# DavidRother/cooking_zoo

Measured on AMD Instinct MI355X. Metric: env-steps/sec at N parallel envs (1/2/4/8 GPU) + achieved HBM GB/s, higher is better.
Workload: dtype u8/u32 state, f64 obs+reward

## Files before the change

### cooking_zoo_amd/_native.py

```python
from __future__ import annotations

import ctypes as C
import os
import sys

_HERE = os.path.dirname(os.path.abspath(__file__))
LIB_PATH = os.environ.get("CZ_LIB", os.path.join(_HERE, "csrc", "libcookingzoo_hip.so"))
HEADER_PATH = os.path.join(os.path.dirname(_HERE), "include", "cookingzoo.h")


def header_abi_version() -> int:
    import re
    if os.path.exists(HEADER_PATH):
        m = re.search(r"^#define\s+CZ_ABI_VERSION\s+(\d+)", open(HEADER_PATH).read(), flags=re.M)
        if not m:
            raise NativeError(f"no CZ_ABI_VERSION in {HEADER_PATH}")
        return int(m.group(1))
    try:
        from cooking_zoo_amd._abi import CZ_ABI_VERSION
    except ImportError as exc:
        raise NativeError(f"neither {HEADER_PATH} nor cooking_zoo_amd/_abi.py (generated by `make -C cooking_zoo_amd/csrc`) is "
                          f"there: the expected ABI number of libcookingzoo_hip.so is unknown") from exc
    return int(CZ_ABI_VERSION)

# ... 82 lines not shown
    ("cz_load_partner_table", C.c_int, [_VP, _VP, _I32]),
    ("cz_load_layout_ranks", C.c_int, [_VP, _I32, _I32, _VP]),
    ("cz_load_goal_table", C.c_int, [_VP, _VP, _I32, _I32]),
    ("cz_num_goals", _I32, [_VP]),
    ("cz_set_tasks_device", C.c_int, [_VP, _VP, _VP, _VP, _I32, _U64]),
    ("cz_set_tasks_refused", _I64, [_VP]),
    ("cz_infos_device", C.c_int, [_VP, _I64, _I64, _VP, _VP, _VP, _VP, _VP]),
    ("cz_num_actions", _I32, [_VP]),
    ("cz_action_effects_device", C.c_int, [_VP, _I64, _I64, _U32, _U32, _VP, _VP]),
    ("cz_render_sprites", _I32, []),
    ("cz_load_sprites", C.c_int, [_VP, _VP, _I32, _I32]),
    ("cz_render_device", C.c_int, [_VP, _I64, _I64, _I32, _U32, _VP, _VP]),
    ("cz_obs_table_f32", C.c_int, [_VP, _VP]),
    ("cz_codes_pitch", _I32, [_VP]),
    ("cz_obs_table", C.c_int, [_VP, _VP]),
    ("cz_obs_table_device", _VP, [_VP]),
    ("cz_probe_closed_loop_compact", C.c_int, [_VP, _I32, _I32, _VP, _VP, _VP, _VP, _VP, C.POINTER(C.c_float)]),
    ("cz_step_device_many", C.c_int, [_VP, _I32, _VP, _I64, _I32, _VP, _VP, _VP, _VP]),
    ("cz_step_device_ring", C.c_int, [_VP, _I32, _VP, _I64, _I32, _I32, _VP, _VP, _VP, _VP]),
    ("cz_ring_prepare", C.c_int, [_VP, _I32, _VP, _I64, _I32, _I32, _VP, _VP, _VP, _VP]),
    ("cz_launch_counts", C.c_int, [_VP, C.POINTER(_I64), C.POINTER(_I64), _I32]),
    ("cz_set_ring_fused", C.c_int, [_VP, _I32]),
    ("cz_ring_fused_steps", C.c_int64, [_VP, _I32]),
    ("cz_last_marks", C.c_int, [_VP, _VP]),
    ("cz_set_stream", C.c_int, [_VP, _VP]),
    ("cz_probe_output_only", C.c_int, [_VP, _VP, C.c_size_t, _I32, _VP]),
    ("cz_probe_policy", C.c_int, [_VP, _VP, _VP, _VP]),
    ("cz_probe_closed_loop", C.c_int, [_VP, _I32, _I32, _VP, _VP, _VP, _VP, _VP, C.POINTER(C.c_float)]),
    ("cz_rollout", C.c_int, [_VP, _I32, _U64, _U32, _VP, _VP, _VP, _VP]),
    ("cz_rollout_compact", C.c_int, [_VP, _I32, _U64, _U32, _VP, _VP, _VP, _VP, _VP]),
    ("cz_rollout_actions", C.c_int, [_VP, _I32, _VP, _VP, _VP, _VP, _VP]),
    ("cz_rollout_f32", C.c_int, [_VP, _I32, _U64, _U32, _VP, _VP, _VP, _VP]),
    ("cz_rollout_actions_f32", C.c_int, [_VP, _I32, _VP, _VP, _VP, _VP, _VP]),
    ("cz_action", _U32, [_U64, _I64, _I32, _U32, _U32]),
    ("cz_next_layout", _U32, [_I64, _U32, _U32, _U32]),
    ("cz_next_layout_group", _U32, [_I64, _U32, _U32, _U32, _U32, _U32]),
    ("cz_dev_alloc", _VP, [_VP, C.c_size_t]),
    ("cz_dev_free", C.c_int, [_VP, _VP]),
    ("cz_host_alloc", _VP, [_VP, C.c_size_t]),
    ("cz_host_free", C.c_int, [_VP, _VP]),
    ("cz_memcpy_h2d", C.c_int, [_VP, _VP, _VP, C.c_size_t]),
    ("cz_memcpy_d2h", C.c_int, [_VP, _VP, _VP, C.c_size_t]),
    ("cz_timer_start", C.c_int, [_VP]),
    ("cz_timer_stop", C.c_int, [_VP, C.POINTER(C.c_float)]),
    ("cz_kernel_time_reset", C.c_int, [_VP, _I32]),
    ("cz_kernel_time_read", C.c_int, [_VP, C.POINTER(C.c_double), C.POINTER(_I64)]),
    ("cz_get_stats", C.c_int, [_VP, C.POINTER(CzStats)]),
    ("cz_reset_stats", C.c_int, [_VP]),
    ("cz_episodes_collect", C.c_int, [_VP, _VP, _VP, _VP, _VP, _VP, _I32, _VP]),
    ("cz_comm_unique_id", C.c_int, [_VP]),
    ("cz_comm_init", C.c_int, [_VP, _I32, _I32, _VP]),
    ("cz_stats_allgather", C.c_int, [_VP, _VP]),
    ("cz_comm_barrier", C.c_int, [_VP]),
    ("cz_runtime_paths", C.c_int, [C.c_char_p, C.c_char_p, C.c_size_t]),
]

ADDED_SYMBOLS = frozenset(["cz_rollout_f32", "cz_rollout_actions_f32", "cz_reset_device", "cz_reset_device_refused",
                           "cz_episodes_collect", "cz_sizeof_episode", "cz_save_device", "cz_restore_device", "cz_restore_device_refused",
                           "cz_observe_grid_device", "cz_grid_channels", "cz_navigate_device", "cz_nav_max_targets", "cz_partner_device",
                           "cz_partner_bad_recipes", "cz_partner_row_words", "cz_load_partner_table", "cz_load_layout_ranks", "cz_num_actions",
                           "cz_action_effects_device", "cz_render_sprites", "cz_load_sprites", "cz_render_device", "cz_load_goal_table", "cz_num_goals",
                           "cz_set_tasks_device", "cz_set_tasks_refused", "cz_infos_device"])

_lib = None
_absent = frozenset()


def _missing(name):
    def call(*args):
        raise NativeError(f"{LIB_PATH} does not export {name}: it was built before that entry point was added - rebuild it "
                          f"(make -C cooking_zoo_amd/csrc)")
    return call


class NativeError(RuntimeError):
    pass


class _LateTorchGuard:

    MESSAGE = ("`import torch` after cooking_zoo_amd has loaded libcookingzoo_hip.so: torch's bundled ROCm runtime would be loaded next "
               "to the system one already in use and the process would abort at exit. Import torch BEFORE creating the first "
               "cooking_zoo_amd environment (see INTEGRATION.md), or set CZ_ALLOW_LATE_TORCH=1 to take the risk.")

    class _Refuse:
# ... 65 lines not shown
```

### cooking_zoo_amd/csrc/cz_api.hip

```cpp
#include <hip/hip_runtime.h>
#include <dlfcn.h>
#include <stdarg.h>
#include <stdio.h>
#include <stdlib.h>
#include <string.h>

#include <atomic>
#include <string>
#include <vector>

#include "../../include/cookingzoo.h"
#include "cz_launch.h"
#include "cz_generate.h"

using namespace cz;

constexpr int STAT_CHAINS = 256, STAT_COLS = 13;
__global__ __launch_bounds__(64) void k_stats_chains(const uint32_t *__restrict__ su, const double *__restrict__ sf,
                                                     const uint32_t *__restrict__ state, int RW, int N,
                                                     unsigned long long *__restrict__ part ) {
    const int chain = (int)blockIdx.x * 4 + ((int)threadIdx.x >> 4), col = (int)threadIdx.x & 15;
    const int widx = col == 0 ? (int)SU_STEPS : col == 1 ? (int)SU_EPISODES : col == 2 ? (int)SU_LENSUM : col == 3 ? (int)SU_TRUNC
                   : col == 4 ? (int)SU_TERM : col < 9 ? (int)SU_COMPLETED0 + col - 5 : 0;
    const int fidx = (col >= 9 && col < STAT_COLS) ? (int)SF_SUM0 + col - 9 : (int)SF_SUM0;
// ... 242 lines not shown
    void *d_sprites = nullptr;
    int32_t sprites_M = 0;
    double obs_table[LUT_SIZE];
    int32_t *d_reset_words = nullptr;
    unsigned long long *d_reset_refused = nullptr;
    unsigned long long *d_restore_refused = nullptr;
    unsigned long long *d_tasks_refused = nullptr;
    uint8_t *d_goal = nullptr;
    int n_goal_rows = 0;
    int num_goals = 0;
    uint8_t *codes = nullptr;
    float *obs32 = nullptr;
    void *d_codes_stage = nullptr;
    void *d_dump = nullptr;
    int32_t *d_actions = nullptr;
    double *d_obs = nullptr;
    char *d_small = nullptr, *h_small = nullptr;
    uint32_t *h_marks = nullptr, *d_marks_mapped = nullptr;
    std::vector<uint32_t> last_marks;
    char *h_stage = nullptr, *d_stage = nullptr;
    struct RingKey {
        const int32_t *ring = nullptr; int64_t stride = 0; int32_t period = 0;
        double *obs = nullptr, *rew = nullptr; uint8_t *term = nullptr, *trunc = nullptr; hipStream_t stream = nullptr; uint64_t version = 0;
        bool operator==(const RingKey &o) const {
            return ring == o.ring && stride == o.stride && period == o.period && obs == o.obs && rew == o.rew && term == o.term &&
                   trunc == o.trunc && stream == o.stream && version == o.version;
        }
    } ring_key;
    struct RunGraph { int32_t slot, len; hipGraphExec_t ge; uint64_t used; };
    std::vector<RunGraph> ring_graphs;
    uint64_t ring_clock = 0;
    int64_t n_graph_kernels = 0, n_direct_kernels = 0;
    uint64_t tables_version = 0;
    hipEvent_t ev0 = nullptr, ev1 = nullptr;
    bool ktime = false;
    std::vector<hipEvent_t> kev;
    size_t kev_used = 0;
    double ktime_ms = 0.0;
    int64_t klaunches = 0;
    void *rccl = nullptr;
    void *comm = nullptr;
    int n_ranks = 1, rank = 0;
    int wt_override = -1;
    bool lean_enabled = true;
    bool lean_cfg_enabled = true;
    int last_step_variant = -1;
    int last_step_lean = -1;
    int last_step_mode = -1;
    bool huge = false;
    int instance = 0;
    unsigned long long *tl_base = nullptr;
    int32_t tl_cap = 0;
    int64_t tl_count = 0;
    bool graphs_enabled = true;
    bool ring_fused = false;
    int64_t n_ring_fused_steps = 0;
    int32_t graph_min_run = 48;
    int32_t ring_prefix = 0;
    size_t zero_copy_bytes = (size_t)256 << 10;
    cz_stats *d_gather = nullptr;
    std::string err;
};

static thread_local std::string g_err;
static int ready(cz_handle h);
static int set_device(cz_handle h);
static int begin_ranged_call(cz_handle h, int64_t b, int64_t c);
static void mark_ranks(cz_handle h, int32_t first, int32_t count, int ok);
static int flush_updates(cz_handle h, bool force);

static int fail(cz_handle h, const char *fmt, ...) {
    char buf[512];
    va_list ap;
    va_start(ap, fmt);
    vsnprintf(buf, sizeof buf, fmt, ap);
    va_end(ap);
    if (h) h->err = buf; else g_err = buf;
    return 1;
}

#define HIPCHK(h, call)                                                                      \
// ... 105 lines not shown
    CREATE_CHK(hipStreamCreateWithFlags(&h->own_stream, hipStreamNonBlocking));
    h->stream = h->own_stream;
    CREATE_CHK(hipEventCreate(&h->ev0));
    CREATE_CHK(hipEventCreate(&h->ev1));
    Params &P = h->P;
    memset(&P, 0, sizeof P);
    P.N = cfg->num_envs; P.A = cfg->num_agents; P.W = cfg->width; P.H = cfg->height; P.D = cfg->max_dyn; P.F = cfg->feat_len;
    const int CW = (C + 3) / 4;
    P.dyn0_off = CELL_WORD0 + CW;
    P.dyn1_off = P.dyn0_off + P.D;
    P.RW = (P.dyn1_off + P.D + 15) / 16 * 16;
    P.scheme = cfg->action_scheme; P.max_steps = cfg->max_steps; P.end_all = cfg->end_condition_all ? 1 : 0;
    P.R = cfg->num_recipes; P.auto_reset = cfg->auto_reset ? 1 : 0; P.env_id_base = cfg->env_id_base;
    P.recipe_reward = cfg->recipe_reward; P.recipe_penalty = cfg->recipe_penalty; P.node_reward = cfg->recipe_node_reward;
    P.time_penalty_step = cfg->max_time_penalty / (double)cfg->max_steps;
    P.T = 1;
    if (const char *s = getenv("CZ_WT")) h->wt_override = atoi(s);
    if (const char *s = getenv("CZ_LEAN")) h->lean_enabled = atoi(s) != 0;
    if (const char *s = getenv("CZ_LEAN_CFG")) h->lean_cfg_enabled = atoi(s) != 0;
    if (const char *s = getenv("CZ_GRAPHS")) h->graphs_enabled = atoi(s) != 0;
    if (const char *s = getenv("CZ_GRAPH_MIN_RUN")) h->graph_min_run = atoi(s) < 4 ? 4 : (atoi(s) > 256 ? 256 : atoi(s));
    if (const char *s = getenv("CZ_RING_PREFIX")) h->ring_prefix = atoi(s) < 0 ? 0 : (atoi(s) > 16 ? 16 : atoi(s));
    if (const char *s = getenv("CZ_ZERO_COPY_BYTES")) h->zero_copy_bytes = (size_t)atoll(s);
#ifdef CZ_SMALL_ONLY
    if (!(P.D <= 64 && C <= 64)) { fail(nullptr, "cz_create: this diagnostic library holds the small kernel instance only"); cz_destroy(h); return 1; }
    h->kl = launchers_small();
#else
    h->instance = (P.D <= 64 && C <= 64) ? 0 : (P.D <= 128 && C <= 256) ? 1 : 2;
    h->kl = h->instance == 0 ? launchers_small() : h->instance == 1 ? launchers_large() : launchers_huge();
#endif
    h->huge = P.D > 128 || C > 256;
    {
        double x = 0.0;
        x += (double)0 * P.node_reward;
        x += 0.0 * P.recipe_reward;
        x += 0.0 * P.recipe_penalty;
        x += P.time_penalty_step;
        P.reward_idle = x;
    }
    const size_t N = (size_t)P.N;
    const size_t state_bytes = N * P.RW * 4;
    CREATE_CHK(hipMalloc(&h->d_state, state_bytes));
    CREATE_CHK(hipMemsetAsync(h->d_state, 0, state_bytes, h->stream));
    CREATE_CHK(hipMalloc(&h->d_stat_u, N * SU_WORDS * 4));
    CREATE_CHK(hipMalloc(&h->d_stat_f, N * SF_WORDS * 8));
    CREATE_CHK(hipMemsetAsync(h->d_stat_u, 0, N * SU_WORDS * 4, h->stream));
// ... 52 lines not shown
        CREATE_CHK(hipMemcpy(h->d_lut, lut, sizeof lut, hipMemcpyHostToDevice));
        CREATE_CHK(hipMemcpy((char *)h->d_lut + sizeof lut, submask, sizeof submask, hipMemcpyHostToDevice));
        P.lut = h->d_lut;
        memcpy(h->obs_table, lut, sizeof lut);
    }
#undef CREATE_CHK
    *out = h;
    return 0;
}

extern "C" int cz_destroy(cz_handle h) {
    if (!h) return 0;
    (void)hipSetDevice(h->cfg.device_id);
    (void)hipStreamSynchronize(h->stream);
    if (h->comm && h->rccl) {
        typedef int (*destroy_t)(void *);
        destroy_t f = (destroy_t)dlsym(h->rccl, "ncclCommDestroy");
        if (f) f(h->comm);
    }
    void *ptrs[] = {h->d_codes_stage, h->d_spawn_tables, h->d_gen_tables, h->d_reset_words, h->d_reset_refused, h->d_restore_refused, h->d_tasks_refused, h->d_goal, h->d_dump, h->d_lut, h->d_sprites, h->d_state, h->d_lay_block, h->d_lay_desc, h->d_lay_rank, h->d_partner, h->d_recipes, h->d_stat_u, h->d_stat_f, h->d_ep_seen, h->d_ep_blocks, h->d_stats_out, h->d_stats_part,
                    h->d_actions, h->d_obs, h->d_small, h->d_gather};
    for (void *p : ptrs)
        if (p) (void)hipFree(p);
    for (auto &r : h->ring_graphs)
        if (r.ge) (void)hipGraphExecDestroy(r.ge);
    if (h->copy_stream) { (void)hipStreamSynchronize(h->copy_stream); (void)hipStreamDestroy(h->copy_stream); }
    if (h->ev_copy_done) (void)hipEventDestroy(h->ev_copy_done);
    if (h->ev_steps_issued) (void)hipEventDestroy(h->ev_steps_issued);
    if (h->ev_main_copy_done) (void)hipEventDestroy(h->ev_main_copy_done);
    if (h->h_lay_stage) (void)hipHostFree(h->h_lay_stage);
    if (h->rank_stream) { (void)hipStreamSynchronize(h->rank_stream); (void)hipStreamDestroy(h->rank_stream); }
    if (h->ev_rank_done) (void)hipEventDestroy(h->ev_rank_done);
    if (h->h_rank_stage) (void)hipHostFree(h->h_rank_stage);
    if (h->h_stage) (void)hipHostFree(h->h_stage);
    if (h->h_small) (void)hipHostFree(h->h_small);
    if (h->h_marks) (void)hipHostFree(h->h_marks);
    for (hipEvent_t e : h->kev) (void)hipEventDestroy(e);
    if (h->ev0) (void)hipEventDestroy(h->ev0);
    if (h->ev1) (void)hipEventDestroy(h->ev1);
    if (h->own_stream) (void)hipStreamDestroy(h->own_stream);
    delete h;
    return 0;
}

extern "C" int cz_set_stream(cz_handle h, void *hip_stream) {
    if (!h) return fail(nullptr, "null handle");
    HIPCHK(h, hipSetDevice(h->cfg.device_id));
    HIPCHK(h, hipStreamSynchronize(h->stream));
    h->stream = hip_stream ? (hipStream_t)hip_stream : h->own_stream;
    h->tables_version++;
    return 0;
}
extern "C" int cz_set_spawn(cz_handle h, double despawn_rate, double respawn_rate, int32_t grace_period, uint64_t seed,
                            int32_t n_levels, const uint8_t *level_of_layout, int32_t stride, const uint8_t *spawn_x, const int32_t *n_x,
                            const uint8_t *spawn_y, const int32_t *n_y) {
// ... 505 lines not shown
        if (c.obs) return "float32 observation rows are switched on (cz_set_f32_output): pass d_obs = NULL, or switch them off "
                          "with cz_set_f32_output(h, NULL) to get float64 rows";
    }
    form = obs32 ? OBS_F32 : codes ? OBS_CODES : OBS_F64;
    P = h->P;
    P.actions = c.actions; P.obs = c.obs; P.rewards = c.rewards; P.term = c.term; P.trunc = c.trunc; P.marks_out = c.marks;
    P.T = c.T; P.seed = c.seed; P.step0 = c.step0;
    if (obs32) P.obs32 = obs32; else P.codes = codes;
    return nullptr;
}

static hipError_t choose_step(cz_handle h, const Params &P, bool fused, ObsForm form, StepChoice &c) {
    c.lean = false;
    c.cfg = -1;
    if (fused && form == OBS_F32) c.mode = P.actions ? ROLLOUT_ACTIONS_F32 : ROLLOUT_F32;
    else if (fused) c.mode = P.actions ? ROLLOUT_ACTIONS : form != OBS_CODES ? ROLLOUT : P.obs ? ROLLOUT_CODES : ROLLOUT_CODES_ONLY;
    else c.mode = form == OBS_F32 ? STEP_F32 : form == OBS_CODES ? STEP_CODES : STEP;
    if (c.mode == STEP)
        c.lean = h->lean_enabled && h->kl.has_lean && P.obs && !P.marks_out && !P.wide && !(P.auto_reset & 2) && P.F <= 128 * OBS_PAIRS && P.wt == 1;
    if (c.lean && h->lean_cfg_enabled) c.cfg = lean_cfg_of(P);
    return !fused && !P.actions ? hipErrorInvalidValue : hipSuccess;
}

static int launch_step(cz_handle h, const StepCall &call) {
    if ((h->P.auto_reset & 2) && h->spawn_layouts != h->n_layouts)
        return fail(h, "despawn / respawn is on, but the layout pool was reloaded since cz_set_spawn (now %d layouts): call cz_set_spawn "
                       "again (it maps every layout to the level whose spawn areas it uses)", h->n_layouts);
    const hipStream_t stream = h->stream;
    const bool fused = call.fused;
    Params P;
    ObsForm form;
    if (const char *refused = resolve_step(h, call, P, form)) return fail(h, "%s", refused);
    const bool f32 = form == OBS_F32;
    const size_t obs_bytes = (size_t)P.N * P.A * P.F * (f32 ? 4 : 8);
    if (!fused) P.wt = obs_bytes > ((size_t)224 << 20) ? 2 : P.N <= 10240 ? 1 : 0;
    else P.wt = (obs_bytes > ((size_t)224 << 20) && (size_t)P.F * (f32 ? 4 : 8) >= 4096) ? 2 : 0;
    if (h->wt_override >= 0) P.wt = h->wt_override;
    if (!fused) {
        if (!P.rewards) P.rewards = (double *)h->d_dump;
        if (!P.term) P.term = (uint8_t *)h->d_dump;
        if (!P.trunc) P.trunc = (uint8_t *)h->d_dump;
    }
#ifdef CZ_TIMELINE
    P.timeline = (h->tl_base && h->tl_cap > 0) ? h->tl_base + (size_t)(h->tl_count++ % h->tl_cap) * (size_t)P.N * 2 : nullptr;
#endif
    hipEvent_t e0 = nullptr, e1 = nullptr;
    if (h->ktime && caller_capturing(h)) return fail(h, "kernel timing (cz_kernel_time_reset) cannot run inside a stream capture of the caller");
    if (h->ktime) {
        while (h->kev.size() < h->kev_used + 2) {
            hipEvent_t e;
            HIPCHK(h, hipEventCreate(&e));
            h->kev.push_back(e);
        }
        e0 = h->kev[h->kev_used]; e1 = h->kev[h->kev_used + 1];
        h->kev_used += 2;
        HIPCHK(h, hipEventRecord(e0, stream));
    }
    StepChoice choice;
    const hipError_t chosen = choose_step(h, P, fused, form, choice);
    h->last_step_lean = choice.lean ? 1 : 0;
    h->last_step_mode = choice.mode;
    h->last_step_variant = !choice.lean ? -1 : choice.cfg < 0 ? 0 : (0x100 | P.R | (P.end_all << 4) | (P.walk_touches << 5));
    HIPCHK(h, chosen);
    HIPCHK(h, h->kl.step(P, stream, choice));
    if (h->ktime) HIPCHK(h, hipEventRecord(e1, stream));
    return 0;
}
extern "C" int cz_reset(cz_handle h, int64_t b, int64_t c, const int32_t *layout_ids, const uint8_t *recipe_ids,
                        const uint32_t *pool_words, double *obs) {
    if (ready(h) || check_range(h, b, c)) return 1;
    if (c == 0) return 0;
    if (!layout_ids || !recipe_ids) return fail(h, "cz_reset: null argument");
    HIPCHK(h, hipSetDevice(h->cfg.device_id));
    std::vector<uint32_t> pools((size_t)c, 0u);
    for (int64_t i = 0; i < c; ++i) {
        if (layout_ids[i] < 0 || layout_ids[i] >= h->n_layouts) return fail(h, "cz_reset: layout id %d out of range", layout_ids[i]);
        for (int r = 0; r < h->P.R; ++r)
            if (recipe_ids[i * 4 + r] >= h->n_recipes) return fail(h, "cz_reset: recipe id %d out of range", recipe_ids[i * 4 + r]);
        if (pool_words) {
            uint32_t base = pool_words[i] & 0xFFFFu, count = pool_words[i] >> 16;
            if (count && (int)(base + count) > h->n_layouts) return fail(h, "cz_reset: layout pool slice [%u,%u) out of range", base, base + count);
            pools[(size_t)i] = pool_words[i];
        }
    }
    int32_t *const d_lay = h->d_reset_words;
    uint32_t *const d_rec = (uint32_t *)h->d_reset_words + h->P.N, *const d_pool = (uint32_t *)h->d_reset_words + 2 * (size_t)h->P.N;
    HIPCHK(h, hipMemcpyAsync(d_lay, layout_ids, (size_t)c * 4, hipMemcpyHostToDevice, h->stream));
// ... 378 lines not shown
extern "C" int cz_diag_read_layout_pool(cz_handle h, int32_t first, int32_t count, uint32_t *records, uint32_t *desc) {
    if (ready(h)) return 1;
    if (!h->d_lay_init || !h->d_lay_desc) return fail(h, "cz_diag_read_layout_pool: no layout pool loaded");
    if (first < 0 || count < 0 || (int64_t)first + count > h->n_layouts)
        return fail(h, "cz_diag_read_layout_pool: slots [%d, %d) outside the resident pool of %d layouts", first, first + count, h->n_layouts);
    if (count == 0) return 0;
    if (set_device(h)) return 1;
    HIPCHK(h, hipStreamSynchronize(h->stream));
    if (records)
        HIPCHK(h, hipMemcpy(records, h->d_lay_init + (size_t)first * h->P.RW, (size_t)count * h->P.RW * 4, hipMemcpyDeviceToHost));
    if (desc)
        HIPCHK(h, hipMemcpy(desc, h->d_lay_desc + (size_t)first * h->P.F, (size_t)count * h->P.F * 4, hipMemcpyDeviceToHost));
    return 0;
}
extern "C" int cz_obs_table(cz_handle h, double *table) {
    if (!h || !table) return fail(h, "cz_obs_table: null argument");
    memcpy(table, h->obs_table, sizeof h->obs_table);
    return 0;
}
extern "C" const void *cz_obs_table_device(cz_handle h) { return h ? (const void *)h->d_lut : nullptr; }

static bool ring_fusable(cz_handle h, const StepCall &c, int32_t K, int64_t stride);
static int launch_ring_fused(cz_handle h, const StepCall &c, int32_t K, const int32_t *d_ring, int64_t stride, int32_t period, int32_t first_slot);
extern "C" int cz_step_device_many(cz_handle h, int32_t K, const int32_t *d_actions, int64_t action_stride, int32_t action_period,
                                   double *d_obs, double *d_rewards, uint8_t *d_term, uint8_t *d_trunc) {
    if (begin_device_call(h, d_actions && K >= 1 && action_period >= 1, "cz_step_device_many: bad arguments")) return 1;
    StepCall c{d_actions, d_obs, d_rewards, d_term, d_trunc};
    if (ring_fusable(h, c, K, action_stride)) return launch_ring_fused(h, c, K, d_actions, action_stride, action_period, 0);
    for (int32_t k = 0; k < K; ++k) {
        c.actions = d_actions + (int64_t)(k % action_period) * action_stride;
        if (launch_step(h, c)) return 1;
    }
    return 0;
}

constexpr int RING_MAX_GRAPH = 256, RING_CACHE = 64;
static int ring_capture(cz_handle h, StepCall &c, const int32_t *d_ring, int64_t stride, int32_t slot, int32_t len, hipGraphExec_t &ge) {
    hipGraph_t g = nullptr;
    HIPCHK(h, hipStreamBeginCapture(h->stream, hipStreamCaptureModeThreadLocal));
    int bad = 0;
    for (int s = 0; s < len && !bad; ++s) {
        c.actions = d_ring + (int64_t)(slot + s) * stride;
        bad = launch_step(h, c);
    }
    const hipError_t ec = hipStreamEndCapture(h->stream, &g);
    if (bad) { if (g) (void)hipGraphDestroy(g); return 1; }
    HIPCHK(h, ec);
    const hipError_t ei = hipGraphInstantiate(&ge, g, nullptr, nullptr, 0);
    (void)hipGraphDestroy(g);
    if (ei != hipSuccess) { ge = nullptr; HIPCHK(h, ei); }
    return 0;
}
static bool ring_select(cz_handle h, const int32_t *d_ring, int64_t stride, int32_t period, double *d_obs, double *d_rewards,
                        uint8_t *d_term, uint8_t *d_trunc) {
    if (h->ktime || !h->graphs_enabled) return false;
    cz_handle_s::RingKey key;
    key.ring = d_ring; key.stride = stride; key.period = period; key.obs = d_obs; key.rew = d_rewards; key.term = d_term;
    key.trunc = d_trunc; key.stream = h->stream; key.version = h->tables_version;
    if (!(key == h->ring_key)) {
        if (!h->ring_graphs.empty()) (void)hipStreamSynchronize(h->stream);
        for (auto &r : h->ring_graphs)
            if (r.ge) (void)hipGraphExecDestroy(r.ge);
        h->ring_graphs.clear();
        h->ring_key = key;
    }
    return true;
}
static int ring_graph(cz_handle h, StepCall &c, const int32_t *d_ring, int64_t stride, int32_t slot, int32_t len, hipGraphExec_t &out) {
    h->ring_clock++;
    for (auto &r : h->ring_graphs)
        if (r.slot == slot && r.len == len) { r.used = h->ring_clock; out = r.ge; return 0; }
    if ((int)h->ring_graphs.size() >= RING_CACHE) {
        size_t victim = 0;
        for (size_t i = 1; i < h->ring_graphs.size(); ++i)
            if (h->ring_graphs[i].used < h->ring_graphs[victim].used) victim = i;
        HIPCHK(h, hipStreamSynchronize(h->stream));
        (void)hipGraphExecDestroy(h->ring_graphs[victim].ge);
        h->ring_graphs.erase(h->ring_graphs.begin() + (long)victim);
    }
    hipGraphExec_t ge = nullptr;
    if (ring_capture(h, c, d_ring, stride, slot, len, ge)) return 1;
    h->ring_graphs.push_back({slot, len, ge, h->ring_clock});
    out = ge;
    return 0;
}
static bool ring_fusable(cz_handle h, const StepCall &c, int32_t K, int64_t stride) {
    Params P;
    ObsForm form;
    return h->ring_fused && K >= 2 && !h->ktime && !resolve_step(h, c, P, form) && form == OBS_F64 && stride == (int64_t)h->P.N * h->P.A;
}
static int launch_ring_fused(cz_handle h, const StepCall &c, int32_t K, const int32_t *d_ring, int64_t stride, int32_t period, int32_t first_slot) {
    const Params &P = h->P;
    const int64_t max_T = (int64_t)(0xFFFFFFFFull / ((uint64_t)P.N * (uint64_t)P.A * 4ull));
    if (max_T < 1) return fail(h, "fused ring run: one action row of %d envs x %d agents exceeds the 4 GiB the kernel addresses", P.N, P.A);
    int32_t k = 0;
    while (k < K) {
        const int32_t slot = (int32_t)(((int64_t)first_slot + k) % period);
        int64_t run = K - k;
        if (run > period - slot) run = period - slot;
        if (run > max_T) run = max_T;
        StepCall q = c;
        q.actions = d_ring + (int64_t)slot * stride;
        q.fused = true; q.T = (int32_t)run; q.seed = 0; q.step0 = 1u;
        if (launch_step(h, q)) return 1;
        k += (int32_t)run;
    }
    h->n_ring_fused_steps += K;
    return 0;
}
static int ring_walk(cz_handle h, int32_t K, const int32_t *d_ring, int64_t stride, int32_t period, int32_t first_slot, double *d_obs,
                     double *d_rewards, uint8_t *d_term, uint8_t *d_trunc, bool launch) {
    StepCall c{d_ring, d_obs, d_rewards, d_term, d_trunc};
    if (ring_fusable(h, c, K, stride)) return launch ? launch_ring_fused(h, c, K, d_ring, stride, period, first_slot) : 0;
    const bool graphs = !caller_capturing(h) && ring_select(h, d_ring, stride, period, d_obs, d_rewards, d_term, d_trunc);
    int32_t k = 0;
    while (k < K) {
        const int32_t slot = (int32_t)(((int64_t)first_slot + k) % period);
        int32_t run = K - k;
        if (run > period - slot) run = period - slot;
        if (run > RING_MAX_GRAPH) run = RING_MAX_GRAPH;
        const int32_t pre = k == 0 ? h->ring_prefix : 0;
        if (graphs && run >= h->graph_min_run + pre) {
            hipGraphExec_t ge = nullptr;
            if (ring_graph(h, c, d_ring, stride, slot + pre, run - pre, ge)) return 1;
            if (launch) {
                for (int32_t j = 0; j < pre; ++j) {
                    c.actions = d_ring + (int64_t)(slot + j) * stride;
                    if (launch_step(h, c)) return 1;
                }
                HIPCHK(h, hipGraphLaunch(ge, h->stream));
                h->n_graph_kernels += run - pre;
                h->n_direct_kernels += pre;
            }
        } else if (launch) {
            for (int32_t j = 0; j < run; ++j) {
                c.actions = d_ring + (int64_t)(slot + j) * stride;
                if (launch_step(h, c)) return 1;
            }
            h->n_direct_kernels += run;
        }
        k += run;
    }
    return 0;
}
extern "C" int cz_ring_prepare(cz_handle h, int32_t K, const int32_t *d_ring, int64_t stride, int32_t period, int32_t first_slot,
                               double *d_obs, double *d_rewards, uint8_t *d_term, uint8_t *d_trunc) {
    if (ready(h)) return 1;
    if (!d_ring || K < 1 || period < 1 || first_slot < 0 || first_slot >= period) return fail(h, "cz_ring_prepare: bad arguments");
    if (set_device(h)) return 1;
    return ring_walk(h, K, d_ring, stride, period, first_slot, d_obs, d_rewards, d_term, d_trunc, false);
}
extern "C" int cz_step_device_ring(cz_handle h, int32_t K, const int32_t *d_ring, int64_t stride, int32_t period, int32_t first_slot,
                                   double *d_obs, double *d_rewards, uint8_t *d_term, uint8_t *d_trunc) {
    if (begin_device_call(h, d_ring && K >= 1 && period >= 1 && first_slot >= 0 && first_slot < period, "cz_step_device_ring: bad arguments")) return 1;
    return ring_walk(h, K, d_ring, stride, period, first_slot, d_obs, d_rewards, d_term, d_trunc, true);
}
extern "C" int cz_set_ring_fused(cz_handle h, int32_t enabled) {
    if (!h) { fail(nullptr, "null handle"); return -1; }
    const int was = h->ring_fused ? 1 : 0;
    h->ring_fused = enabled != 0;
    return was;
}
extern "C" int64_t cz_ring_fused_steps(cz_handle h, int32_t reset) {
    if (!h) return 0;
    const int64_t n = h->n_ring_fused_steps;
    if (reset) h->n_ring_fused_steps = 0;
    return n;
}
extern "C" int cz_launch_counts(cz_handle h, int64_t *graph_kernels, int64_t *direct_kernels, int32_t reset) {
    if (!h) return fail(nullptr, "null handle");
    if (graph_kernels) *graph_kernels = h->n_graph_kernels;
    if (direct_kernels) *direct_kernels = h->n_direct_kernels;
    if (reset) h->n_graph_kernels = h->n_direct_kernels = 0;
    return 0;
}

extern "C" int cz_rollout(cz_handle h, int32_t T, uint64_t seed, uint32_t step0, double *d_obs, double *d_rewards,
                          uint8_t *d_term, uint8_t *d_trunc) {
    if (begin_device_call(h, T >= 1, "cz_rollout: T must be >= 1", "cz_rollout", T)) return 1;
    StepCall c{nullptr, d_obs, d_rewards, d_term, d_trunc};
    c.fused = true; c.T = T; c.seed = seed; c.step0 = step0;
    return launch_step(h, c);
}

extern "C" int cz_rollout_compact(cz_handle h, int32_t T, uint64_t seed, uint32_t step0, uint8_t *d_codes, double *d_obs, double *d_rewards,
// ... 430 lines not shown
```

### cooking_zoo_amd/sharded.py

```python
from __future__ import annotations

import ctypes as C
import json
import threading
from concurrent.futures import ThreadPoolExecutor
from typing import Dict, List, Optional, Sequence, Tuple

import numpy as np

from cooking_zoo_amd import _native, effects as _effects
from cooking_zoo_amd import distributed as czd
from cooking_zoo_amd.vec_env import BatchTables, CookingVecEnv


class ShardedBuffer:

    def __init__(self, owner: "ShardedVecEnv", leading: Tuple[int, ...], per_env: Tuple[int, ...], dtype):
        self.owner, self.leading, self.per_env, self.dtype = owner, tuple(leading), tuple(per_env), np.dtype(dtype)
        self.axis = len(self.leading)
        self.parts = owner._each(lambda i, env: env.alloc(self.leading + (env.num_envs,) + self.per_env, self.dtype))

    def to_host(self) -> np.ndarray:
        return np.concatenate(self.owner._each(lambda i, env: self.parts[i].to_host()), axis=self.axis)

# ... 383 lines not shown
        def one(i, env, first_slot):
            _, h, a, o = fixed[i]
            check(h, ring(h, *a, first_slot, *o))
            check(h, sync(h))
            env._advance(a[0])

        if len(fixed) == 1:
            env0 = fixed[0][0]
            return lambda first_slot: one(0, env0, int(first_slot))
        return lambda first_slot: self._each(lambda i, env: one(i, env, int(first_slot)))

    def ring_prepare(self, K, d_ring, action_period, first_slot, d_obs, d_rewards, d_term, d_trunc):
        P = self._part
        from cooking_zoo_amd.vec_env import _dev_ptr as p

        def prep(i, env):
            _native.check(env._h, _native.lib().cz_ring_prepare(env._h, int(K), p(P(d_ring, i)), env.num_envs * env.num_agents, int(action_period),
                                                                int(first_slot), p(P(d_obs, i)), p(P(d_rewards, i)), p(P(d_term, i)), p(P(d_trunc, i))))
        self._each(prep)

    def set_ring_fused(self, enabled=True):
        return self._each(lambda i, env: env.set_ring_fused(enabled))[0]

    def rollout(self, T, seed, step0=0, d_obs=None, d_rewards=None, d_term=None, d_trunc=None):
        P = self._part
        self._each(lambda i, env: env.rollout(T, seed, step0, P(d_obs, i), P(d_rewards, i), P(d_term, i), P(d_trunc, i)))

    def rollout_compact(self, T, seed, step0, d_codes, d_obs=None, d_rewards=None, d_term=None, d_trunc=None):
        P = self._part
        self._each(lambda i, env: env.rollout_compact(T, seed, step0, P(d_codes, i), P(d_obs, i), P(d_rewards, i), P(d_term, i), P(d_trunc, i)))

    def rollout_actions(self, d_actions, T, d_obs=None, d_rewards=None, d_term=None, d_trunc=None):
        P = self._part
        self._each(lambda i, env: env.rollout_actions(P(d_actions, i), T, P(d_obs, i), P(d_rewards, i), P(d_term, i), P(d_trunc, i)))

    def rollout_f32(self, T, seed, step0, d_obs32, d_rewards=None, d_term=None, d_trunc=None):
        P = self._part
        self._each(lambda i, env: env.rollout_f32(T, seed, step0, P(d_obs32, i), P(d_rewards, i), P(d_term, i), P(d_trunc, i)))

    def rollout_actions_f32(self, d_actions, T, d_obs32, d_rewards=None, d_term=None, d_trunc=None):
        P = self._part
        self._each(lambda i, env: env.rollout_actions_f32(P(d_actions, i), T, P(d_obs32, i), P(d_rewards, i), P(d_term, i), P(d_trunc, i)))

    def sync(self):
        self._each(lambda i, env: env.sync())

# ... 54 lines not shown
```

### cooking_zoo_amd/vec_env.py

```python
from __future__ import annotations

import contextlib
import ctypes as C
import random as _random

import numpy as np

from cooking_zoo_amd import _native, effects as _effects, grid as _grid, nav as _nav, partner as _partner, render as _render, rotation as _rotation, soa, tasks as _tasks
from cooking_zoo_amd.cooking_book import recipe_drawer
from cooking_zoo_amd.cooking_world.actions import ACTION_SCHEMES
from cooking_zoo_amd.cooking_world.engine import load_level as _ll
from cooking_zoo_amd.cooking_world.layout import feature_length

DEFAULT_REWARD_SCHEME = {"recipe_reward": 20, "max_time_penalty": -5, "recipe_penalty": -40, "recipe_node_reward": 0}


def _ptr(a):
    return a.ctypes.data_as(C.c_void_p) if a is not None else None


class DeviceBuffer:

    def __init__(self, env, shape, dtype):
        self.env, self.shape, self.dtype = env, tuple(int(s) for s in shape), np.dtype(dtype)
# ... 605 lines not shown
        shape = (n, self.num_agents, self.num_actions)
        noop = np.zeros(shape, np.uint8)
        noop[..., 0] = 1
        if n == 0:
            return noop, np.zeros(shape, np.uint8)
        with self._scratch((shape, np.uint8, noop), (shape, np.uint8, np.zeros(shape, np.uint8))) as (d_m, d_e):
            self.action_effects_device(d_m, d_e, agents=agents, ignore=ignore, env_begin=env_begin, env_count=n)
            return d_m.to_host(), d_e.to_host()

    def alloc(self, shape, dtype):
        b = DeviceBuffer(self, shape, dtype)
        self._buffers.append(b)
        return b

    def set_ring_fused(self, enabled=True):
        rc = _native.lib().cz_set_ring_fused(self._h, 1 if enabled else 0)
        if rc < 0:
            raise _native.NativeError((_native.lib().cz_last_error(self._h) or b"cz_set_ring_fused failed").decode())
        return bool(rc)

    def ring_fused_steps(self, reset=False):
        return int(_native.lib().cz_ring_fused_steps(self._h, 1 if reset else 0))

    def set_stream(self, stream=None):
        raw = getattr(stream, "cuda_stream", stream)
        raw = getattr(raw, "value", raw)
        _native.check(self._h, _native.lib().cz_set_stream(self._h, C.c_void_p(int(raw)) if raw else None))
        self._caller_stream = bool(raw)

    def step_device(self, d_actions, d_obs, d_rewards, d_term, d_trunc):
        p = _dev_ptr
        _native.check(self._h, _native.lib().cz_step_device(self._h, p(d_actions), p(d_obs), p(d_rewards), p(d_term),
                                                            p(d_trunc)))
        self._issued(1)

    def step_device_compact(self, d_actions, d_codes, d_rewards, d_term, d_trunc, d_obs=None):
        p = _dev_ptr
        _native.check(self._h, _native.lib().cz_step_device_compact(self._h, p(d_actions), p(d_codes), p(d_obs), p(d_rewards), p(d_term),
                                                                    p(d_trunc)))
        self._issued(1)

    def reset_device(self, d_mask=None, d_layout_ids=None, d_obs=None, d_obs32=None, d_codes=None):
        p = _dev_ptr
        _native.check(self._h, _native.lib().cz_reset_device(self._h, p(d_mask), p(d_layout_ids), p(d_obs), p(d_obs32), p(d_codes)))

    def reset_device_refused(self):
# ... 195 lines not shown
```

### include/cookingzoo.h

```cpp
#ifndef COOKINGZOO_H
#define COOKINGZOO_H

#include <stddef.h>
#include <stdint.h>

#ifdef __cplusplus
extern "C" {
#endif

#define CZ_ABI_VERSION 10

typedef struct cz_handle_s *cz_handle;

typedef struct cz_config {
    int32_t num_envs;
    int32_t num_agents;
    int32_t width, height;
    int32_t max_dyn;
    int32_t feat_len;
    int32_t action_scheme;
    int32_t max_steps;
    int32_t end_condition_all;
    int32_t num_recipes;
    int32_t auto_reset;
// ... 130 lines not shown
                           uint8_t *d_terminations, uint8_t *d_truncations);
int cz_set_compact_output(cz_handle h, uint8_t *d_codes);
int cz_step_compact(cz_handle h, const int32_t *actions, uint8_t *codes, double *rewards, uint8_t *terminations, uint8_t *truncations);
int32_t cz_codes_pitch(cz_handle h);
int cz_obs_table(cz_handle h, double table[256]);
const void *cz_obs_table_device(cz_handle h);

int cz_step_device_f32(cz_handle h, const int32_t *d_actions, float *d_obs32, double *d_rewards, uint8_t *d_terminations,
                       uint8_t *d_truncations);
int cz_set_f32_output(cz_handle h, float *d_obs32);
int cz_obs_table_f32(cz_handle h, float table[256]);

int cz_step_device_many(cz_handle h, int32_t K, const int32_t *d_actions, int64_t action_stride, int32_t action_period,
                        double *d_obs, double *d_rewards, uint8_t *d_terminations, uint8_t *d_truncations);

int cz_step_device_ring(cz_handle h, int32_t K, const int32_t *d_ring, int64_t action_stride, int32_t action_period,
                        int32_t first_slot, double *d_obs, double *d_rewards, uint8_t *d_terminations, uint8_t *d_truncations);

int cz_ring_prepare(cz_handle h, int32_t K, const int32_t *d_ring, int64_t action_stride, int32_t action_period,
                    int32_t first_slot, double *d_obs, double *d_rewards, uint8_t *d_terminations, uint8_t *d_truncations);

int cz_set_ring_fused(cz_handle h, int32_t enabled);
int64_t cz_ring_fused_steps(cz_handle h, int32_t reset);

int cz_launch_counts(cz_handle h, int64_t *graph_kernels, int64_t *direct_kernels, int32_t reset);

int cz_rollout(cz_handle h, int32_t T, uint64_t seed, uint32_t step0, double *d_obs, double *d_rewards,
               uint8_t *d_terminations, uint8_t *d_truncations);

int cz_rollout_compact(cz_handle h, int32_t T, uint64_t seed, uint32_t step0, uint8_t *d_codes, double *d_obs, double *d_rewards,
                       uint8_t *d_terminations, uint8_t *d_truncations);

int cz_rollout_actions(cz_handle h, int32_t T, const int32_t *d_actions, double *d_obs, double *d_rewards,
                       uint8_t *d_terminations, uint8_t *d_truncations);

int cz_rollout_f32(cz_handle h, int32_t T, uint64_t seed, uint32_t step0, float *d_obs32, double *d_rewards,
                   uint8_t *d_terminations, uint8_t *d_truncations);
int cz_rollout_actions_f32(cz_handle h, int32_t T, const int32_t *d_actions, float *d_obs32, double *d_rewards,
                           uint8_t *d_terminations, uint8_t *d_truncations);

uint32_t cz_action(uint64_t seed, int64_t env_global, int32_t agent, uint32_t step, uint32_t n_actions);
uint32_t cz_next_layout(int64_t env_global, uint32_t episode, uint32_t pool_word, uint32_t n_layouts);
uint32_t cz_next_layout_group(int64_t env_global, uint32_t episode, uint32_t pool_word, uint32_t n_layouts, uint32_t groups,
                              uint32_t active);

void *cz_dev_alloc(cz_handle h, size_t bytes);
// ... 31 lines not shown
```

Measured before the change: 762.6 million.

## Split ring step graphs across two streams by env halves

Divides the env batch into two halves aligned to workgroup size and captures a separate step graph for each half, launching them on the main stream and a new side stream joined by fork/join events. Automatic mode turns this on only for mid-sized N (4096–32768) on instance 0, so two independent step chains can run concurrently on the GPU rather than serially. A small sleep kernel staggers the second graph. It costs extra graph memory and event synchronisation, and adds risk on setups with few hardware queues.

```diff
diff --git a/cooking_zoo_amd/_native.py b/cooking_zoo_amd/_native.py
--- a/cooking_zoo_amd/_native.py
+++ b/cooking_zoo_amd/_native.py
@@ -128,6 +128,8 @@
     ("cz_launch_counts", C.c_int, [_VP, C.POINTER(_I64), C.POINTER(_I64), _I32]),
     ("cz_set_ring_fused", C.c_int, [_VP, _I32]),
     ("cz_ring_fused_steps", C.c_int64, [_VP, _I32]),
+    ("cz_set_ring_split", C.c_int, [_VP, _I32]),
+    ("cz_ring_split_parts", _I32, [_VP]),
     ("cz_last_marks", C.c_int, [_VP, _VP]),
     ("cz_set_stream", C.c_int, [_VP, _VP]),
     ("cz_probe_output_only", C.c_int, [_VP, _VP, C.c_size_t, _I32, _VP]),
@@ -166,7 +168,7 @@
                            "cz_observe_grid_device", "cz_grid_channels", "cz_navigate_device", "cz_nav_max_targets", "cz_partner_device",
                            "cz_partner_bad_recipes", "cz_partner_row_words", "cz_load_partner_table", "cz_load_layout_ranks", "cz_num_actions",
                            "cz_action_effects_device", "cz_render_sprites", "cz_load_sprites", "cz_render_device", "cz_load_goal_table", "cz_num_goals",
-                           "cz_set_tasks_device", "cz_set_tasks_refused", "cz_infos_device"])
+                           "cz_set_tasks_device", "cz_set_tasks_refused", "cz_infos_device", "cz_set_ring_split", "cz_ring_split_parts"])
 
 _lib = None
 _absent = frozenset()
diff --git a/cooking_zoo_amd/csrc/cz_api.hip b/cooking_zoo_amd/csrc/cz_api.hip
--- a/cooking_zoo_amd/csrc/cz_api.hip
+++ b/cooking_zoo_amd/csrc/cz_api.hip
@@ -288,12 +288,13 @@
     struct RingKey {
         const int32_t *ring = nullptr; int64_t stride = 0; int32_t period = 0;
         double *obs = nullptr, *rew = nullptr; uint8_t *term = nullptr, *trunc = nullptr; hipStream_t stream = nullptr; uint64_t version = 0;
+        int32_t parts = 1;
         bool operator==(const RingKey &o) const {
             return ring == o.ring && stride == o.stride && period == o.period && obs == o.obs && rew == o.rew && term == o.term &&
-                   trunc == o.trunc && stream == o.stream && version == o.version;
+                   trunc == o.trunc && stream == o.stream && version == o.version && parts == o.parts;
         }
     } ring_key;
-    struct RunGraph { int32_t slot, len; hipGraphExec_t ge; uint64_t used; };
+    struct RunGraph { int32_t slot, len; hipGraphExec_t ge, ge2; uint64_t used; };
     std::vector<RunGraph> ring_graphs;
     uint64_t ring_clock = 0;
     int64_t n_graph_kernels = 0, n_direct_kernels = 0;
@@ -323,6 +324,10 @@
     int64_t n_ring_fused_steps = 0;
     int32_t graph_min_run = 48;
     int32_t ring_prefix = 0;
+    int32_t ring_split = -1;
+    bool few_queues = false;
+    hipStream_t split_stream = nullptr;
+    hipEvent_t ev_fork = nullptr, ev_join = nullptr;
     size_t zero_copy_bytes = (size_t)256 << 10;
     cz_stats *d_gather = nullptr;
     std::string err;
@@ -474,6 +479,8 @@
     if (const char *s = getenv("CZ_GRAPH_MIN_RUN")) h->graph_min_run = atoi(s) < 4 ? 4 : (atoi(s) > 256 ? 256 : atoi(s));
     if (const char *s = getenv("CZ_RING_PREFIX")) h->ring_prefix = atoi(s) < 0 ? 0 : (atoi(s) > 16 ? 16 : atoi(s));
     if (const char *s = getenv("CZ_ZERO_COPY_BYTES")) h->zero_copy_bytes = (size_t)atoll(s);
+    if (const char *s = getenv("CZ_RING_SPLIT")) h->ring_split = atoi(s) == 2 ? 2 : atoi(s) == 0 ? 0 : -1;
+    if (const char *s = getenv("GPU_MAX_HW_QUEUES")) h->few_queues = atoi(s) < 4;
 #ifdef CZ_SMALL_ONLY
     if (!(P.D <= 64 && C <= 64)) { fail(nullptr, "cz_create: this diagnostic library holds the small kernel instance only"); cz_destroy(h); return 1; }
     h->kl = launchers_small();
@@ -572,8 +579,10 @@
                     h->d_actions, h->d_obs, h->d_small, h->d_gather};
     for (void *p : ptrs)
         if (p) (void)hipFree(p);
-    for (auto &r : h->ring_graphs)
+    for (auto &r : h->ring_graphs) {
         if (r.ge) (void)hipGraphExecDestroy(r.ge);
+        if (r.ge2) (void)hipGraphExecDestroy(r.ge2);
+    }
     if (h->copy_stream) { (void)hipStreamSynchronize(h->copy_stream); (void)hipStreamDestroy(h->copy_stream); }
     if (h->ev_copy_done) (void)hipEventDestroy(h->ev_copy_done);
     if (h->ev_steps_issued) (void)hipEventDestroy(h->ev_steps_issued);
@@ -581,6 +590,9 @@
     if (h->h_lay_stage) (void)hipHostFree(h->h_lay_stage);
     if (h->rank_stream) { (void)hipStreamSynchronize(h->rank_stream); (void)hipStreamDestroy(h->rank_stream); }
     if (h->ev_rank_done) (void)hipEventDestroy(h->ev_rank_done);
+    if (h->split_stream) { (void)hipStreamSynchronize(h->split_stream); (void)hipStreamDestroy(h->split_stream); }
+    if (h->ev_fork) (void)hipEventDestroy(h->ev_fork);
+    if (h->ev_join) (void)hipEventDestroy(h->ev_join);
     if (h->h_rank_stage) (void)hipHostFree(h->h_rank_stage);
     if (h->h_stage) (void)hipHostFree(h->h_stage);
     if (h->h_small) (void)hipHostFree(h->h_small);
@@ -1132,7 +1144,34 @@
     return !fused && !P.actions ? hipErrorInvalidValue : hipSuccess;
 }
 
-static int launch_step(cz_handle h, const StepCall &call) {
+static Params sub_range(const Params &P, ObsForm form, int32_t begin, int32_t count) {
+    Params Q = P;
+    const size_t b = (size_t)begin, row = (size_t)P.A * (size_t)P.F;
+    Q.N = count;
+    Q.env_id_base = P.env_id_base + begin;
+    Q.state = P.state + b * (size_t)P.RW;
+    if (P.actions) Q.actions = P.actions + b * (size_t)P.A;
+    if (P.obs) Q.obs = P.obs + b * row;
+    if (P.rewards) Q.rewards = P.rewards + b * (size_t)P.A;
+    if (P.term) Q.term = P.term + b * (size_t)P.A;
+    if (P.trunc) Q.trunc = P.trunc + b * (size_t)P.A;
+    if (P.marks_out) Q.marks_out = P.marks_out + b * 2;
+    if (form == OBS_F32) Q.obs32 = P.obs32 + b * row;
+    else if (P.codes) Q.codes = P.codes + b * (size_t)P.A * (size_t)codes_pitch(P.F);
+    Q.stat_u = P.stat_u + b * SU_WORDS;
+    Q.stat_f = P.stat_f + b * SF_WORDS;
+#ifdef CZ_PROFILE
+    if (P.stamps) Q.stamps = P.stamps + b * 16;
+#endif
+#ifdef CZ_TIMELINE
+    if (P.timeline) Q.timeline = P.timeline + b * 2;
+#endif
+    return Q;
+}
+
+struct RunSplit { int32_t begin1; hipStream_t side; int only = -1; };
+
+static int launch_step(cz_handle h, const StepCall &call, const RunSplit *split = nullptr) {
     if ((h->P.auto_reset & 2) && h->spawn_layouts != h->n_layouts)
         return fail(h, "despawn / respawn is on, but the layout pool was reloaded since cz_set_spawn (now %d layouts): call cz_set_spawn "
                        "again (it maps every layout to the level whose spawn areas it uses)", h->n_layouts);
@@ -1172,7 +1211,10 @@
     h->last_step_mode = choice.mode;
     h->last_step_variant = !choice.lean ? -1 : choice.cfg < 0 ? 0 : (0x100 | P.R | (P.end_all << 4) | (P.walk_touches << 5));
     HIPCHK(h, chosen);
-    HIPCHK(h, h->kl.step(P, stream, choice));
+    if (split && !fused) {
+        if (split->only != 1) HIPCHK(h, h->kl.step(sub_range(P, form, 0, split->begin1), stream, choice));
+        if (split->only != 0) HIPCHK(h, h->kl.step(sub_range(P, form, split->begin1, P.N - split->begin1), split->side, choice));
+    } else HIPCHK(h, h->kl.step(P, stream, choice));
     if (h->ktime) HIPCHK(h, hipEventRecord(e1, stream));
     return 0;
 }
@@ -1597,28 +1639,85 @@
 
 static bool ring_fusable(cz_handle h, const StepCall &c, int32_t K, int64_t stride);
 static int launch_ring_fused(cz_handle h, const StepCall &c, int32_t K, const int32_t *d_ring, int64_t stride, int32_t period, int32_t first_slot);
+
+constexpr int32_t RING_SPLIT_MIN_N = 4096, RING_SPLIT_MAX_N = 32768;
+enum : int { SPLIT_GRAPHS = 1, SPLIT_DIRECT = 2 };
+static int run_split(cz_handle h, bool capturing) {
+    if (h->ring_split == 0 || capturing || h->ktime || h->few_queues || h->P.N < 2) return 0;
+    if (h->ring_split == 2) return SPLIT_GRAPHS | SPLIT_DIRECT;
+    return h->instance == 0 && h->P.N >= RING_SPLIT_MIN_N && h->P.N <= RING_SPLIT_MAX_N ? SPLIT_GRAPHS : 0;
+}
+static int split_begin(cz_handle h, RunSplit &s) {
+    const int32_t N = h->P.N, epw = h->instance == 2 ? envs_per_wg<16>() : envs_per_wg<1>(), half = (N + 1) / 2;
+    const int32_t whole = (half + epw - 1) / epw * epw;
+    s.begin1 = whole < N ? whole : half;
+    if (!h->split_stream) {
+        HIPCHK(h, hipStreamCreateWithFlags(&h->split_stream, hipStreamNonBlocking));
+        HIPCHK(h, hipEventCreateWithFlags(&h->ev_fork, hipEventDisableTiming));
+        HIPCHK(h, hipEventCreateWithFlags(&h->ev_join, hipEventDisableTiming));
+    }
+    s.side = h->split_stream;
+    return 0;
+}
+static int split_fork(cz_handle h) {
+    HIPCHK(h, hipEventRecord(h->ev_fork, h->stream));
+    HIPCHK(h, hipStreamWaitEvent(h->split_stream, h->ev_fork, 0));
+    return 0;
+}
+static int split_join(cz_handle h) {
+    HIPCHK(h, hipEventRecord(h->ev_join, h->split_stream));
+    HIPCHK(h, hipStreamWaitEvent(h->stream, h->ev_join, 0));
+    return 0;
+}
+#ifndef CZ_RING_DELAY_SLEEPS
+#define CZ_RING_DELAY_SLEEPS 12
+#endif
+__global__ __launch_bounds__(64) void k_ring_delay() {
+#pragma unroll
+    for (int i = 0; i < CZ_RING_DELAY_SLEEPS; ++i) __builtin_amdgcn_s_sleep(16);
+}
+static int launch_slots(cz_handle h, StepCall &c, const int32_t *d_ring, int64_t stride, int32_t slot, int32_t count, const RunSplit *split) {
+    if (count < 1) return 0;
+    if (split && split_fork(h)) return 1;
+    int bad = 0;
+    for (int32_t j = 0; j < count && !bad; ++j) {
+        c.actions = d_ring + (int64_t)(slot + j) * stride;
+        bad = launch_step(h, c, split);
+    }
+    if (split && split_join(h)) return 1;
+    return bad;
+}
 extern "C" int cz_step_device_many(cz_handle h, int32_t K, const int32_t *d_actions, int64_t action_stride, int32_t action_period,
                                    double *d_obs, double *d_rewards, uint8_t *d_term, uint8_t *d_trunc) {
     if (begin_device_call(h, d_actions && K >= 1 && action_period >= 1, "cz_step_device_many: bad arguments")) return 1;
     StepCall c{d_actions, d_obs, d_rewards, d_term, d_trunc};
     if (ring_fusable(h, c, K, action_stride)) return launch_ring_fused(h, c, K, d_actions, action_stride, action_period, 0);
-    for (int32_t k = 0; k < K; ++k) {
+    RunSplit split;
+    const bool two = (run_split(h, caller_capturing(h)) & SPLIT_DIRECT) != 0;
+    if (two && (split_begin(h, split) || split_fork(h))) return 1;
+    int bad = 0;
+    for (int32_t k = 0; k < K && !bad; ++k) {
         c.actions = d_actions + (int64_t)(k % action_period) * action_stride;
-        if (launch_step(h, c)) return 1;
-    }
-    return 0;
+        bad = launch_step(h, c, two ? &split : nullptr);
+    }
+    if (two && split_join(h)) return 1;
+    return bad;
 }
 
 constexpr int RING_MAX_GRAPH = 256, RING_CACHE = 64;
-static int ring_capture(cz_handle h, StepCall &c, const int32_t *d_ring, int64_t stride, int32_t slot, int32_t len, hipGraphExec_t &ge) {
+static int ring_capture(cz_handle h, StepCall &c, const int32_t *d_ring, int64_t stride, int32_t slot, int32_t len, hipStream_t on,
+                        const RunSplit *split, int part, hipGraphExec_t &ge) {
+    RunSplit one;
+    if (split) { one = *split; one.only = part; }
     hipGraph_t g = nullptr;
-    HIPCHK(h, hipStreamBeginCapture(h->stream, hipStreamCaptureModeThreadLocal));
+    HIPCHK(h, hipStreamBeginCapture(on, hipStreamCaptureModeThreadLocal));
+    if (part == 1 && CZ_RING_DELAY_SLEEPS > 0) hipLaunchKernelGGL(k_ring_delay, dim3(1), dim3(64), 0, on);
     int bad = 0;
     for (int s = 0; s < len && !bad; ++s) {
         c.actions = d_ring + (int64_t)(slot + s) * stride;
-        bad = launch_step(h, c);
-    }
-    const hipError_t ec = hipStreamEndCapture(h->stream, &g);
+        bad = launch_step(h, c, split ? &one : nullptr);
+    }
+    const hipError_t ec = hipStreamEndCapture(on, &g);
     if (bad) { if (g) (void)hipGraphDestroy(g); return 1; }
     HIPCHK(h, ec);
     const hipError_t ei = hipGraphInstantiate(&ge, g, nullptr, nullptr, 0);
@@ -1626,37 +1725,45 @@
     if (ei != hipSuccess) { ge = nullptr; HIPCHK(h, ei); }
     return 0;
 }
+static void ring_drop(cz_handle h) {
+    if (!h->ring_graphs.empty()) (void)hipStreamSynchronize(h->stream);
+    for (auto &r : h->ring_graphs) {
+        if (r.ge) (void)hipGraphExecDestroy(r.ge);
+        if (r.ge2) (void)hipGraphExecDestroy(r.ge2);
+    }
+    h->ring_graphs.clear();
+}
 static bool ring_select(cz_handle h, const int32_t *d_ring, int64_t stride, int32_t period, double *d_obs, double *d_rewards,
-                        uint8_t *d_term, uint8_t *d_trunc) {
+                        uint8_t *d_term, uint8_t *d_trunc, int32_t parts) {
     if (h->ktime || !h->graphs_enabled) return false;
     cz_handle_s::RingKey key;
     key.ring = d_ring; key.stride = stride; key.period = period; key.obs = d_obs; key.rew = d_rewards; key.term = d_term;
-    key.trunc = d_trunc; key.stream = h->stream; key.version = h->tables_version;
+    key.trunc = d_trunc; key.stream = h->stream; key.version = h->tables_version; key.parts = parts;
     if (!(key == h->ring_key)) {
-        if (!h->ring_graphs.empty()) (void)hipStreamSynchronize(h->stream);
-        for (auto &r : h->ring_graphs)
-            if (r.ge) (void)hipGraphExecDestroy(r.ge);
-        h->ring_graphs.clear();
+        ring_drop(h);
         h->ring_key = key;
     }
     return true;
 }
-static int ring_graph(cz_handle h, StepCall &c, const int32_t *d_ring, int64_t stride, int32_t slot, int32_t len, hipGraphExec_t &out) {
+static int ring_graph(cz_handle h, StepCall &c, const int32_t *d_ring, int64_t stride, int32_t slot, int32_t len, const RunSplit *split,
+                      hipGraphExec_t &out, hipGraphExec_t &out2) {
     h->ring_clock++;
     for (auto &r : h->ring_graphs)
-        if (r.slot == slot && r.len == len) { r.used = h->ring_clock; out = r.ge; return 0; }
+        if (r.slot == slot && r.len == len) { r.used = h->ring_clock; out = r.ge; out2 = r.ge2; return 0; }
     if ((int)h->ring_graphs.size() >= RING_CACHE) {
         size_t victim = 0;
         for (size_t i = 1; i < h->ring_graphs.size(); ++i)
             if (h->ring_graphs[i].used < h->ring_graphs[victim].used) victim = i;
         HIPCHK(h, hipStreamSynchronize(h->stream));
         (void)hipGraphExecDestroy(h->ring_graphs[victim].ge);
+        if (h->ring_graphs[victim].ge2) (void)hipGraphExecDestroy(h->ring_graphs[victim].ge2);
         h->ring_graphs.erase(h->ring_graphs.begin() + (long)victim);
     }
-    hipGraphExec_t ge = nullptr;
-    if (ring_capture(h, c, d_ring, stride, slot, len, ge)) return 1;
-    h->ring_graphs.push_back({slot, len, ge, h->ring_clock});
-    out = ge;
+    hipGraphExec_t ge = nullptr, ge2 = nullptr;
+    if (ring_capture(h, c, d_ring, stride, slot, len, h->stream, split, split ? 0 : -1, ge)) return 1;
+    if (split && ring_capture(h, c, d_ring, stride, slot, len, split->side, split, 1, ge2)) { (void)hipGraphExecDestroy(ge); return 1; }
+    h->ring_graphs.push_back({slot, len, ge, ge2, h->ring_clock});
+    out = ge; out2 = ge2;
     return 0;
 }
 static bool ring_fusable(cz_handle h, const StepCall &c, int32_t K, int64_t stride) {
@@ -1687,7 +1794,12 @@
                      double *d_rewards, uint8_t *d_term, uint8_t *d_trunc, bool launch) {
     StepCall c{d_ring, d_obs, d_rewards, d_term, d_trunc};
     if (ring_fusable(h, c, K, stride)) return launch ? launch_ring_fused(h, c, K, d_ring, stride, period, first_slot) : 0;
-    const bool graphs = !caller_capturing(h) && ring_select(h, d_ring, stride, period, d_obs, d_rewards, d_term, d_trunc);
+    const bool capturing = caller_capturing(h);
+    RunSplit two;
+    const int parts = run_split(h, capturing);
+    const RunSplit *const split = parts & SPLIT_GRAPHS ? &two : nullptr, *const split_direct = parts & SPLIT_DIRECT ? &two : nullptr;
+    if (parts && split_begin(h, two)) return 1;
+    const bool graphs = !capturing && ring_select(h, d_ring, stride, period, d_obs, d_rewards, d_term, d_trunc, split ? 2 : 1);
     int32_t k = 0;
     while (k < K) {
         const int32_t slot = (int32_t)(((int64_t)first_slot + k) % period);
@@ -1696,22 +1808,21 @@
         if (run > RING_MAX_GRAPH) run = RING_MAX_GRAPH;
         const int32_t pre = k == 0 ? h->ring_prefix : 0;
         if (graphs && run >= h->graph_min_run + pre) {
-            hipGraphExec_t ge = nullptr;
-            if (ring_graph(h, c, d_ring, stride, slot + pre, run - pre, ge)) return 1;
+            hipGraphExec_t ge = nullptr, ge2 = nullptr;
+            if (ring_graph(h, c, d_ring, stride, slot + pre, run - pre, split, ge, ge2)) return 1;
             if (launch) {
-                for (int32_t j = 0; j < pre; ++j) {
-                    c.actions = d_ring + (int64_t)(slot + j) * stride;
-                    if (launch_step(h, c)) return 1;
+                if (launch_slots(h, c, d_ring, stride, slot, pre, split_direct)) return 1;
+                if (ge2 && split_fork(h)) return 1;
+                HIPCHK(h, hipGraphLaunch(ge, h->stream));
+                if (ge2) {
+                    HIPCHK(h, hipGraphLaunch(ge2, h->split_stream));
+                    if (split_join(h)) return 1;
                 }
-                HIPCHK(h, hipGraphLaunch(ge, h->stream));
                 h->n_graph_kernels += run - pre;
                 h->n_direct_kernels += pre;
             }
         } else if (launch) {
-            for (int32_t j = 0; j < run; ++j) {
-                c.actions = d_ring + (int64_t)(slot + j) * stride;
-                if (launch_step(h, c)) return 1;
-            }
+            if (launch_slots(h, c, d_ring, stride, slot, run, split_direct)) return 1;
             h->n_direct_kernels += run;
         }
         k += run;
@@ -1736,6 +1847,20 @@
     h->ring_fused = enabled != 0;
     return was;
 }
+extern "C" int cz_set_ring_split(cz_handle h, int32_t mode) {
+    if (!h) { fail(nullptr, "null handle"); return -2; }
+    if (mode != -1 && mode != 0 && mode != 2) { fail(h, "cz_set_ring_split: mode %d is none of -1 (automatic), 0 (off), 2 (two parts)", mode); return -2; }
+    const int was = h->ring_split;
+    if (mode != was && !caller_capturing(h)) {
+        if (hipSetDevice(h->cfg.device_id) != hipSuccess) { fail(h, "cz_set_ring_split: hipSetDevice failed"); return -2; }
+        ring_drop(h);
+    }
+    h->ring_split = mode;
+    h->tables_version++;
+    return was;
+}
+extern "C" int32_t cz_ring_split_parts(cz_handle h) { return h ? (run_split(h, false) ? 2 : 1) : 0; }
+extern "C" int32_t cz_diag_ring_graphs(cz_handle h) { return h ? (int32_t)h->ring_graphs.size() : 0; }
 extern "C" int64_t cz_ring_fused_steps(cz_handle h, int32_t reset) {
     if (!h) return 0;
     const int64_t n = h->n_ring_fused_steps;
diff --git a/cooking_zoo_amd/sharded.py b/cooking_zoo_amd/sharded.py
--- a/cooking_zoo_amd/sharded.py
+++ b/cooking_zoo_amd/sharded.py
@@ -429,6 +429,9 @@
     def set_ring_fused(self, enabled=True):
         return self._each(lambda i, env: env.set_ring_fused(enabled))[0]
 
+    def set_ring_split(self, mode=-1):
+        return self._each(lambda i, env: env.set_ring_split(mode))[0]
+
     def rollout(self, T, seed, step0=0, d_obs=None, d_rewards=None, d_term=None, d_trunc=None):
         P = self._part
         self._each(lambda i, env: env.rollout(T, seed, step0, P(d_obs, i), P(d_rewards, i), P(d_term, i), P(d_trunc, i)))
diff --git a/cooking_zoo_amd/vec_env.py b/cooking_zoo_amd/vec_env.py
--- a/cooking_zoo_amd/vec_env.py
+++ b/cooking_zoo_amd/vec_env.py
@@ -651,6 +651,15 @@
     def ring_fused_steps(self, reset=False):
         return int(_native.lib().cz_ring_fused_steps(self._h, 1 if reset else 0))
 
+    def set_ring_split(self, mode=-1):
+        rc = _native.lib().cz_set_ring_split(self._h, int(mode))
+        if rc < -1:
+            raise _native.NativeError((_native.lib().cz_last_error(self._h) or b"cz_set_ring_split failed").decode())
+        return int(rc)
+
+    def ring_split_parts(self):
+        return int(_native.lib().cz_ring_split_parts(self._h))
+
     def set_stream(self, stream=None):
         raw = getattr(stream, "cuda_stream", stream)
         raw = getattr(raw, "value", raw)
diff --git a/include/cookingzoo.h b/include/cookingzoo.h
--- a/include/cookingzoo.h
+++ b/include/cookingzoo.h
@@ -176,6 +176,9 @@
 
 int cz_set_ring_fused(cz_handle h, int32_t enabled);
 int64_t cz_ring_fused_steps(cz_handle h, int32_t reset);
+
+int cz_set_ring_split(cz_handle h, int32_t mode);
+int32_t cz_ring_split_parts(cz_handle h);
 
 int cz_launch_counts(cz_handle h, int64_t *graph_kernels, int64_t *direct_kernels, int32_t reset);
 
```

New measurement: 780.3 million (median of 6 runs). 2.3% higher.
